# ZhenlongYuan/DVP-MVS

Hardware: AMD Instinct MI355X
Metric: Mpixels/sec/PatchMatch-iteration (higher is better)
Workload: dtype f32

## Files before the change

__graft_entry__.py:

```python
import importlib
import os
import subprocess
import sys

ROOT = os.path.dirname(os.path.abspath(__file__))
if ROOT not in sys.path:
    sys.path.insert(0, ROOT)


def build() -> None:
    subprocess.check_call(["make", "-s", "-C", os.path.join(ROOT, "dvp-mvs_amd", "csrc")])
    host = os.path.join(ROOT, "dvp-mvs_amd", "host")
    if os.path.exists(os.path.join(host, "Makefile")):
        subprocess.check_call(["make", "-s", "-C", host])
    subprocess.check_call(["make", "-s", "-C", os.path.join(ROOT, "oracle")])
    subprocess.check_call(["make", "-s", "-C", os.path.join(ROOT, "tests", "emul")])
    subprocess.check_call(["make", "-s", "-C", os.path.join(ROOT, "tests", "sweep_host")])
    subprocess.check_call(["make", "-s", "-C", os.path.join(ROOT, "tests", "host")])
    subprocess.check_call(["make", "-s", "-C", os.path.join(ROOT, "tests", "half16")])
    subprocess.check_call(["make", "-s", "-C", os.path.join(ROOT, "tests", "jpeg_host")])
    subprocess.check_call(["make", "-s", "-C", os.path.join(ROOT, "tests", "edges_host")])
    subprocess.check_call(["make", "-s", "-C", os.path.join(ROOT, "tests", "viewclean_host")])
    subprocess.check_call(["make", "-s", "-C", os.path.join(ROOT, "tests", "labels_host")])
    subprocess.check_call(["make", "-s", "-C", os.path.join(ROOT, "tests", "pyramid_host")])
    subprocess.check_call(["make", "-s", "-C", os.path.join(ROOT, "tests", "prior_host")])
    subprocess.check_call(["make", "-s", "-C", os.path.join(ROOT, "tests", "reuse_host")])
    subprocess.check_call(["make", "-s", "-C", os.path.join(ROOT, "tests", "devmem_host")])
    subprocess.check_call(["make", "-s", "-C", os.path.join(ROOT, "tests", "jpeg_dec_host")])
    subprocess.check_call(["make", "-s", "-C", os.path.join(ROOT, "tests", "convert_host")])
    subprocess.check_call(["make", "-s", "-C", os.path.join(ROOT, "tests", "undistort_host")])
    subprocess.check_call(["make", "-s", "-C", os.path.join(ROOT, "tests", "cloudeval_host")])
    pkg = importlib.import_module("dvp-mvs_amd")
    lib = pkg.get_capi().lib()
    missing = [s for s in pkg.get_capi().EXPORTS + pkg.get_capi().EXPORTS_WITH_DIGITS if not hasattr(lib, s)]
    if missing:
        raise RuntimeError("libdvp_mvs_hip.so lacks symbols: %s" % missing)


def smoke() -> None:
    import numpy as np
    pkg = importlib.import_module("dvp-mvs_amd")
    synth, capi = pkg.synth, pkg.get_capi()
    from oracle import oracle as O
    W, H, S = 96, 64, 3
    sc = synth.make_scene(W, H, S)
    p = synth.default_params(S + 1, max_iterations=1, state=synth.FIRST_INIT, use_APD=0)
    p["depth_min"] = np.float32(2.5) * np.float32(0.6)
    p["depth_max"] = np.float32(6.5) * np.float32(1.2)
    state = dict(planes=np.zeros((H * W, 4), np.float32), edge=sc["edge"], label=sc["label"],
                 radius=np.full(H * W, 5, np.int32))
# ... 21 lines not shown
```

dvp-mvs_amd/csrc/dvp_ctx.hpp:

```cpp
#ifndef DVP_CTX_HPP_
#define DVP_CTX_HPP_

#include "dvp_jpeg_enc.h"
#include "dvp_edges_run.h"
#include "dvp_viewclean_run.h"
#include "dvp_prior_run.h"
#include <cstdlib>
#include <string>
#include <vector>
#include <cstdio>
#include <mutex>
#include <condition_variable>
#include <initializer_list>

struct EventPair { int stage; hipEvent_t a, b; };
enum { EV_TOTAL = -1, EV_ITER_LOOP = -2 };

struct dvp_ctx {
	int device = 0;
	FormSwitches sw;
	int W = 0, H = 0, NI = 0, pitch = 0;
	size_t L = 0;
	hipStream_t stream = nullptr;
	bool cand_mask_fits = true;
	uint8_t* cand_mask = nullptr;
	unsigned *cand_list = nullptr, *cand_n = nullptr;
	uint32_t* sel_snap = nullptr;
	hipStream_t side = nullptr;
	hipEvent_t side_fork = nullptr, side_join = nullptr;
	Dev d{};
	std::vector<void*> allocs;
	float* images = nullptr;
	uint8_t* images8 = nullptr;
	int* images8_flag = nullptr;
	bool images8_ok = false;
	uint32_t* images16 = nullptr;
	bool images16_ok = false;
	float* image_stage = nullptr;
	float* depths = nullptr;
	uint32_t* edge_bits = nullptr;
	uint32_t* strong_bits = nullptr;
	uint32_t* strong_bits_t = nullptr;
	int* edge_sat = nullptr;
	DvpCamera* cameras = nullptr; ViewConst* views = nullptr; int* sector_taps = nullptr; int* sector_start = nullptr;
	f4* planes = nullptr; f4* planes_snap = nullptr; f4* fit_planes = nullptr;
	int* search_pos = nullptr;
	float* slot_costs = nullptr;
	float* strong_rec = nullptr;
	float* reuse_costs = nullptr; PlaneKey* reuse_keys = nullptr; ReuseHdr* reuse_hdr = nullptr;
	bool reuse_fits = true;
	uint32_t reuse_epoch = 0;
	bool split_fits = true;
	f4* sweep_rec = nullptr; float* sweep_cost = nullptr; float* sweep_pc = nullptr;
	bool sweep_fits = true;
	int sweep_band_rows = 0;
	float* costs = nullptr; float* costs_snap = nullptr; float* complex_ = nullptr;
	uint32_t* selected_views = nullptr;
	uint8_t* view_weight = nullptr; uint8_t* weak_info = nullptr; uint8_t* weak_reliable = nullptr; uint8_t* edge = nullptr;
	s2* label_stop = nullptr; s2* weak_nearest_strong = nullptr; s2* neighbours = nullptr; s2* gn_points = nullptr; int* gn_count = nullptr; s2* candidate = nullptr; s2* edge_neigh = nullptr; s2* label_boundary = nullptr;
	int* neighbours_map = nullptr; int* label = nullptr; int* radius = nullptr;
	unsigned long long* eval_counter = nullptr;
	float* scratch_out = nullptr;
	size_t weak_alloc = 0;
	AnchorRec* anchor_tab = nullptr;
	size_t anchor_tab_alloc = 0;
	bool anchor_tab_valid = false;
	bool anchor_tab_fits = true;
	WeakRec* weak_rec = nullptr; f2* weak_ctab = nullptr; float* weak_ev = nullptr;
	size_t weak_phase_alloc = 0;
	bool weak_phase_fits = true;
	int* weak_list = nullptr;
	size_t weak_list_alloc = 0;
	int* weak_counts = nullptr;
	int* weak_totals_host = nullptr;
	uint8_t* coarse = nullptr;
	uint8_t* maps_out = nullptr;
	hipStream_t copy = nullptr;
	uint8_t* maps_host = nullptr;
	std::mutex dl_m;
	std::condition_variable dl_cv;
	bool dl_busy = false;
	bool dl_fetching = false;
	size_t coarse_alloc = 0;
	uint8_t* pv_bgr[3] = { nullptr, nullptr, nullptr };
	dvpjpeg::Encoder pv_enc[3];
	unsigned long long* pv_total = nullptr;
	hipEvent_t pv_done = nullptr;
	hipStream_t pv_copy = nullptr;
// ... 52 lines not shown
		if (c->allocs[i] == (void*)*p) { c->allocs[i] = c->allocs.back(); c->allocs.pop_back(); break; }
	(void)hipFree((void*)*p);
	*p = nullptr;
}

struct AllocReq { void** p; size_t bytes; bool zero; };
template <class T>
static AllocReq areq(T** p, size_t bytes, bool zero = false) { return { reinterpret_cast<void**>(p), bytes, zero }; }

static void bump_reuse_epoch(dvp_ctx* c) {
	if (++c->reuse_epoch == 0) {
		if (c->reuse_hdr) (void)hipMemsetAsync(c->reuse_hdr, 0, c->L * sizeof(ReuseHdr), c->stream);
		c->reuse_epoch = 1;
	}
	c->d.reuse_epoch = c->reuse_epoch;
}

static size_t img16_plane_bytes(int W, int H) { return (size_t)img16_tiles_x(W) * img16_tiles_y(H) * 128; }

static bool anchor_table_off(const dvp_ctx* c) { return c->sw.anchor_tab_off || !c->anchor_tab_fits; }

static void sync_dev_struct(dvp_ctx* c) {
	Dev& d = c->d;
	d.width = c->W; d.height = c->H; d.num_images = c->NI; d.pitch = c->pitch;
	d.org = kImgPad * c->pitch + kImgPad;
	d.plane_stride = (size_t)c->pitch * (c->H + 2 * kImgPad);
	d.images = c->images; d.images8 = c->images8_ok ? c->images8 : nullptr; d.img8_tiles_x = img8_tiles_x(c->W); d.img8_plane_bytes = (size_t)img8_tiles_x(c->W) * img8_tiles_y(c->H) * 128;
	d.images16 = c->images16_ok ? c->images16 : nullptr; d.img16_tiles_x = img16_tiles_x(c->W); d.img16_plane_bytes = img16_plane_bytes(c->W, c->H);
	d.depths = c->depths; d.cameras = c->cameras; d.views = c->views; d.sector_taps = c->sector_taps; d.sector_start = c->sector_start;
	d.search_pos = c->search_pos;
	d.sweep_px0 = 0; d.sweep_row0 = 0; d.sweep_row1 = 0;
	d.sweep_all_slots = c->sw.sweep_all_slots ? 1 : 0;
	d.sweep_rec = c->sweep_rec; d.sweep_cost = c->sweep_cost; d.sweep_pc = c->sweep_pc; d.slot_costs = c->slot_costs; d.strong_rec = c->strong_rec; d.half_w = (c->W + 1) / 2;
	d.reuse_costs = c->reuse_costs; d.reuse_keys = c->reuse_keys; d.reuse_hdr = c->reuse_hdr; d.reuse_epoch = c->reuse_epoch;
	d.planes = c->planes; d.planes_snap = c->planes_snap; d.costs = c->costs; d.costs_snap = c->costs_snap;
	d.selected_views = c->selected_views; d.view_weight = c->view_weight; d.weak_info = c->weak_info;
	d.weak_reliable = c->weak_reliable; d.weak_nearest_strong = c->weak_nearest_strong;
	d.anchor_tab = (anchor_table_off(c) || !c->anchor_tab_valid) ? nullptr : c->anchor_tab; d.neighbours_map = c->neighbours_map; d.neighbours = c->neighbours; d.gn_points = c->gn_points; d.gn_count = c->gn_count; d.fit_planes = c->fit_planes;
	d.candidate = c->candidate; d.edge = c->edge; d.edge_bits = c->edge_bits; d.strong_bits = c->strong_bits; d.strong_bits_t = c->strong_bits_t; d.edge_sat = c->edge_sat; d.sat_cells_x = sat_cells(c->W); d.sat_cells_y = sat_cells(c->H); d.edge_tiles_x = edge_tiles_x(c->W); d.edge_neigh = c->edge_neigh; d.label = c->label;
	d.label_boundary = c->label_boundary; d.label_stop = c->label_stop; d.complex_ = c->complex_; d.radius = c->radius;
	d.weak_list = c->weak_list;
	d.weak_rec = c->weak_rec; d.weak_ctab = c->weak_ctab; d.weak_ev = c->weak_ev;
	d.eval_counter = c->profiling ? c->eval_counter : nullptr;
}

static int ensure_images16(dvp_ctx* c) {
	if (c->images16) return 0;
	return dalloc(c, &c->images16, img16_plane_bytes(c->W, c->H) / 4 * c->NI, false);
}

static int set_device(dvp_ctx* c) {
	HIP_TRY(c, hipSetDevice(c->device));
	return 0;
}

static size_t alloc_group_or_fall_back(dvp_ctx* c, std::initializer_list<AllocReq> reqs, const char* hook, bool* fits, const char* msg, double gb, size_t retry_bytes = 0) {
	void* got[4] = { nullptr, nullptr, nullptr, nullptr };
	const AllocReq* r = reqs.begin();
	const size_t n = reqs.size();
	size_t first = r[0].bytes;
	bool ok = n <= 4 && !(hook && getenv(hook));
	for (size_t i = 0; i < n && ok; ++i) {
		if (!r[i].p) continue;
		ok = hipMalloc(&got[i], r[i].bytes) == hipSuccess;
		if (!ok && i == 0 && retry_bytes) { (void)hipGetLastError(); first = retry_bytes; ok = hipMalloc(&got[0], first) == hipSuccess; }
		if (!ok) got[i] = nullptr;
// ... 22 lines not shown
```

dvp-mvs_amd/csrc/dvp_dev.hpp:

```cpp
#ifndef DVP_DEV_HPP_
#define DVP_DEV_HPP_

#include <stdint.h>
#include <math.h>
#include <float.h>
#include <string.h>
#include "../../include/dvp_mvs.h"
#include "dvp_forms.hpp"

#if defined(__HIPCC__)
#include <hip/hip_runtime.h>
#define DVP_HD __host__ __device__ __forceinline__
#define DVP_HD_NOINLINE __host__ __device__ __noinline__
#else
#define DVP_HD inline
#define DVP_HD_NOINLINE inline
#endif
#ifndef DVP_STREAM_HINTS
#define DVP_STREAM_HINTS 3
#endif
#if defined(__HIP_DEVICE_COMPILE__)
#define DVP_NT_STORE(bit, p, v) do { if ((DVP_STREAM_HINTS) & (bit)) __builtin_nontemporal_store((v), (p)); else *(p) = (v); } while (0)
#define DVP_NT_LOAD(bit, p) (((DVP_STREAM_HINTS) & (bit)) ? __builtin_nontemporal_load(p) : *(p))
#else
// ... 60 lines not shown
	f4* planes;
	const f4* planes_snap;
	float* costs;
	const float* costs_snap;
	uint32_t* selected_views;
	uint8_t* view_weight;
	uint8_t* weak_info;
	uint8_t* weak_reliable;
	s2* weak_nearest_strong;
	const int* neighbours_map;
	s2* neighbours;
	s2* gn_points;
	int* gn_count;
	f4* fit_planes;
	s2* candidate;
	AnchorRec* anchor_tab;
	WeakRec* weak_rec;
	f2* weak_ctab;
	float* weak_ev;
	const uint8_t* edge;
	int* search_pos;
	float* slot_costs;
	float* strong_rec;
	float* reuse_costs;
	PlaneKey* reuse_keys;
	ReuseHdr* reuse_hdr;
	uint32_t reuse_epoch;
	f4* sweep_rec;
	float* sweep_cost;
	float* sweep_pc;
	int sweep_px0;
	int sweep_row0, sweep_row1;
	int sweep_all_slots;
	int half_w;
	uint32_t* edge_bits;
	int edge_tiles_x;
	uint32_t* strong_bits;
	uint32_t* strong_bits_t;
	int* edge_sat;
	int sat_cells_x, sat_cells_y;
	s2* edge_neigh;
	const int* label;
	s2* label_boundary;
	s2* label_stop;
	float* complex_;
	int* radius;
	const int* weak_list;
	int weak_black, weak_red;
	unsigned long long* eval_counter;
};

#define DVP_MIN(a, b) ((a) > (b) ? (b) : (a))
#define DVP_MAX(a, b) ((a) < (b) ? (b) : (a))

DVP_HD float dvp_expf(float x) {
	if (!(x > -103.0f)) return (x != x) ? x : 0.0f;
	if (x > 88.72f) return INFINITY;
	const float n = rintf(x * 1.44269504088896341f);
	float r = fmaf(n, -0.693359375f, x);
	r = fmaf(n, 2.12194440e-4f, r);
	float p = 1.9875691500e-4f;
	p = fmaf(p, r, 1.3981999507e-3f);
	p = fmaf(p, r, 8.3334519073e-3f);
	p = fmaf(p, r, 4.1665795894e-2f);
	p = fmaf(p, r, 1.6666665459e-1f);
	p = fmaf(p, r, 5.0000001201e-1f);
// ... 543 lines not shown
```

dvp-mvs_amd/csrc/dvp_engine.hip:

```cpp
#include "dvp_kernels.hpp"
#include "dvp_ctx.hpp"
#ifdef DVP_PROBE
#include "dvp_probe.inc"
#endif
#include "dvp_pyramid_run.h"
#include <cstring>
#include <thread>
#include <chrono>
#include <algorithm>
#include <cmath>

extern "C" {

int dvp_ctx_create(int device, int width, int height, int num_images, dvp_ctx** out) {
	if (!out) return 1;
	*out = nullptr;
	if (width <= 0 || height <= 0 || num_images < 2 || num_images > DVP_MAX_IMAGES || width > 32767 || height > 32767) {
		g_create_error = "dvp_ctx_create: bad dimensions (2 <= num_images <= 32, sizes <= 32767: short2 pixel coordinates)";
		return 1;
	}
	{
		const unsigned long long pitch = ((unsigned long long)width + 2 * kImgPad + 63) / 64 * 64;
		if (pitch * ((unsigned long long)height + 2 * kImgPad) * 8ull >= (1ull << 32)) {
			g_create_error = "dvp_ctx_create: image too large (a padded row-pair plane must stay below 4 GiB)";
// ... 499 lines not shown
	if (alloc_group_or_fall_back(c, { areq(&c->weak_rec, cap * sizeof(WeakRec)), areq(&c->weak_ctab, cap * kTaps * kTaps * sizeof(f2)), areq(&c->weak_ev, cap * 8 * S * sizeof(float)) },
			"DVP_TEST_WEAK_PHASE_ALLOC_FAIL", &c->weak_phase_fits, "dvp: no room for the phased weak update's hand-over buffers (%.2f GB); using the one-wave kernel\n", (double)cap * (sizeof(WeakRec) + 288 + 32 * S) / 1e9))
		c->weak_phase_alloc = cap;
	return 0;
}

static void ensure_strong_reuse_buffers(dvp_ctx* c) {
	if (c->reuse_costs || !c->sw.strong_reuse || !c->reuse_fits || strong_form(c->sw, c->NI - 1, c->split_fits, false, 0).kernel != STRONG_SPLIT) return;
	const size_t L = c->L, vec = (size_t)kSlotCount * (c->NI - 1) * L * sizeof(float) + 64 ;
	const size_t Lh = (size_t)((c->W + 1) / 2) * c->H;
	alloc_group_or_fall_back(c, { areq(&c->reuse_costs, vec), areq(&c->reuse_keys, L * kSlotCount * sizeof(PlaneKey)), areq(&c->reuse_hdr, L * sizeof(ReuseHdr), true),
			c->strong_rec ? AllocReq{} : areq(&c->strong_rec, (size_t)SR_FIELDS * Lh * sizeof(*c->strong_rec)) },
		"DVP_TEST_REUSE_ALLOC_FAIL", &c->reuse_fits, "dvp: no room for the strong update's plane cache (%.1f GB); every visit evaluates all its planes\n", (double)(vec + L * (kSlotCount * sizeof(PlaneKey) + sizeof(ReuseHdr))) / 1e9);
}
static void ensure_strong_split_buffers(dvp_ctx* c) {
	if (c->slot_costs || strong_form(c->sw, c->NI - 1, c->split_fits, false, 0).kernel != STRONG_SPLIT) return;
	if (!getenv("DVP_TEST_SPLIT_ALLOC_FAIL")) {
		ensure_strong_reuse_buffers(c);
		if (c->reuse_costs) return;
	}
	const size_t Lh = (size_t)((c->W + 1) / 2) * c->H;
	alloc_group_or_fall_back(c, { areq(&c->slot_costs, (size_t)kSlotCount * (c->NI - 1) * Lh * sizeof(*c->slot_costs) + 64 ),
			areq(&c->strong_rec, (size_t)SR_FIELDS * Lh * sizeof(*c->strong_rec)) },
		"DVP_TEST_SPLIT_ALLOC_FAIL", &c->split_fits, "dvp: no room for the split strong update's cost buffer (%.1f GB); using the monolithic kernel\n", (double)kSlotCount * (c->NI - 1) * Lh * 4 / 1e9);
}
static void ensure_sweep_buffers(dvp_ctx* c) {
	if (c->sweep_cost || !c->sw.sweep_split || !c->sweep_fits) return;
	const size_t L = c->L;
	c->sweep_band_rows = sweep_band_rows(c->sw, c->W, c->H, c->NI - 1);
	const size_t band_px = c->sweep_band_rows > 0 ? (size_t)c->sweep_band_rows * c->W : L;
	alloc_group_or_fall_back(c, { areq(&c->sweep_rec, 2 * L * sizeof(f4)), areq(&c->sweep_pc, 61 * L * sizeof(float)), areq(&c->sweep_cost, sweep_cost_floats(band_px, c->NI - 1) * sizeof(float)) },
		"DVP_TEST_SWEEP_ALLOC_FAIL", &c->sweep_fits, "dvp: no room for the view-compacted DepthToWeak's cost buffer (%.1f GB); using the fused kernel\n", (double)(c->NI - 1) * kSweepFields * L * 4 / 1e9);
}


#define DVP_PICK(NAME, SUF) (c->d.sampler ? NAME##_exact##SUF : NAME##SUF)
#define DVP_PICK_FMT(NAME, TAIL) (fmt == 1 ? DVP_PICK(NAME, _u8##TAIL) : (fmt == 2 ? DVP_PICK(NAME, _f16##TAIL) : DVP_PICK(NAME, TAIL)))

static LaunchArgs make_args(const LaunchGeom& g, int colour, int iter) {
	LaunchArgs a;
	a.tiles_x = g.tiles_x; a.tiles = g.tiles; a.rows = g.rows; a.half = g.half ? 1 : 0;
	a.colour = colour; a.iter = iter;
	return a;
}

static void launch_gen_candidates(dvp_ctx* c, hipStream_t stream, const Dev& d, unsigned blocks, const LaunchArgs& a, const unsigned* list = nullptr, const unsigned* n_list = nullptr) {
	const bool all = gen_candidates_all_views(d);
	const dim3 grid(blocks, all ? (unsigned)((c->NI - 1 + kCandGroup - 1) / kCandGroup) : (unsigned)(c->NI - 1)), block(256);
	if (list) hipLaunchKernelGGL(all ? dvp_gen_candidates_views_list : dvp_gen_candidates_list, grid, block, 0, stream, d, list, n_list);
	else hipLaunchKernelGGL(all ? dvp_gen_candidates_views : dvp_gen_candidates, grid, block, 0, stream, d, a);
}

static int launch_strong_prep(dvp_ctx* c, const LaunchGeom& g, const LaunchArgs& a) {
	EventPair prep;
	prep.stage = DVP_ST_STRONG_PREP;
	HIP_TRY(c, hipEventCreate(&prep.a));
	HIP_TRY(c, hipEventCreate(&prep.b));
	HIP_TRY(c, hipEventRecord(prep.a, c->stream));
	HIP_TRY(c, hipMemcpyAsync(c->planes_snap, c->planes, c->L * 16, hipMemcpyDeviceToDevice, c->stream));
	HIP_TRY(c, hipMemcpyAsync(c->costs_snap, c->costs, c->L * 4, hipMemcpyDeviceToDevice, c->stream));
	ensure_strong_split_buffers(c);
	hipLaunchKernelGGL(dvp_strong_search, dim3(g.grid()), dim3(256), 0, c->stream, c->d, a);
	if (strong_form(c->sw, c->NI - 1, c->split_fits, c->d.reuse_hdr != nullptr, 0).plan) hipLaunchKernelGGL(dvp_strong_plan, dim3(g.grid()), dim3(256), 0, c->stream, c->d, a);
	HIP_TRY(c, hipGetLastError());
	HIP_TRY(c, hipEventRecord(prep.b, c->stream));
	c->events.push_back(prep);
// ... 72 lines not shown
	if (stage == DVP_ST_FIND_NEAREST_STRONG) HIP_TRY(c, hipMemsetAsync(c->weak_nearest_strong, 0xFF, c->L * sizeof(s2), c->stream));
	if (stage == DVP_ST_RANSAC_FIT) HIP_TRY(c, hipMemcpyAsync(c->fit_planes, c->planes, c->L * 16, hipMemcpyDeviceToDevice, c->stream));
	ListArgs la;
	la.iter = iter;
	la.covered_rows = 2 * make_geom(c->W, c->H, true).rows;
	la.base = (stage == DVP_ST_WEAK_UPDATE && colour == 1) ? c->d.weak_black : 0;
	la.count = (stage == DVP_ST_WEAK_UPDATE) ? (colour == 0 ? c->d.weak_black : (colour == 1 ? c->d.weak_red : c->d.weak_black + c->d.weak_red)) : c->d.weak_black + c->d.weak_red;
	if (la.count <= 0) return 0;
	const dim3 lg((la.count + 255) / 256);
	switch (stage) {
	case DVP_ST_FIND_NEAREST_STRONG: hipLaunchKernelGGL(DVP_PICK(dvp_find_nearest_strong_list, ), lg, block, 0, c->stream, c->d, la); break;
	case DVP_ST_GEN_NEIGHBOURS:
		if (c->sw.gn_wave) hipLaunchKernelGGL(dvp_gen_neighbours_search, dim3((la.count + 3) / 4), block, 0, c->stream, c->d, la);
		else hipLaunchKernelGGL(dvp_gen_neighbours_list, lg, block, 0, c->stream, c->d, la);
		hipLaunchKernelGGL(dvp_gen_neighbours_fit, dim3(la.count), dim3(64), 0, c->stream, c->d, la);
		break;
	case DVP_ST_NEIGHBOUR_UPDATE: hipLaunchKernelGGL(DVP_PICK(dvp_neighbour_update_list, ), lg, block, 0, c->stream, c->d, la); break;
	case DVP_ST_RANSAC_FIT:
		if (c->sw.ransac_wave) hipLaunchKernelGGL(dvp_ransac_fit_plane_wave, dim3(la.count), dim3(64), 0, c->stream, c->d, la);
		else hipLaunchKernelGGL(DVP_PICK(dvp_ransac_fit_plane_list, ), lg, block, 0, c->stream, c->d, la);
		break;
	case DVP_ST_WEAK_UPDATE:
		if (launch_weak_update(c, la)) return 1;
		break;
	}
	HIP_TRY(c, hipGetLastError());
	return 0;
}

static int launch_sweeps(dvp_ctx* c, const LaunchGeom& g, const LaunchArgs& a, bool fused) {
	const dim3 grid(g.grid()), block(256);
	if (sweep_form(c->sw, fused, c->d.params, c->sweep_fits, c->W, c->H).kernel == SWEEP_PASSES) ensure_sweep_buffers(c);
	const SweepForm f = sweep_form(c->sw, fused, c->d.params, c->sweep_fits, c->W, c->H);
	if (f.kernel == SWEEP_PASSES) {
		LaunchArgs s0 = a, s1 = a, sb = a;
		s0.iter = 0; s1.iter = 1; sb.iter = kSweepBorderOnly;
		const int etx = (c->W + 63) / 64, ety = (c->H + kSweepRows - 1) / kSweepRows;
		s0.tiles_x = s1.tiles_x = etx; s0.tiles = s1.tiles = etx * ety;
		const dim3 egrid((unsigned)(etx * ety), (unsigned)(c->NI - 1));
		hipLaunchKernelGGL(dvp_sweep_prepare, grid, block, 0, c->stream, c->d, a);
		const int band_rows = c->sweep_band_rows > 0 ? c->sweep_band_rows : c->H;
		for (int row0 = 0; row0 < c->H; row0 += band_rows) {
			Dev db = c->d;
			LaunchArgs b0 = s0, b1 = s1;
			dim3 bgrid = egrid;
			b0.rows = b1.rows = 0;
			if (c->sweep_band_rows > 0) {
				const int row1 = std::min(c->H, row0 + band_rows);
				db.sweep_px0 = row0 * c->W; db.sweep_row0 = row0; db.sweep_row1 = row1;
				const int bty = (row1 - row0 + kSweepRows - 1) / kSweepRows;
				b0.rows = b1.rows = row0 / kSweepRows;
				b0.tiles = b1.tiles = etx * bty;
				bgrid = dim3((unsigned)(etx * bty), (unsigned)(c->NI - 1));
			}
			const auto eval = c->sw.sweep_all_slots ? DVP_PICK(dvp_sweep_eval, _all) : DVP_PICK(dvp_sweep_eval, );
			hipLaunchKernelGGL(eval, bgrid, dim3(64), 0, c->stream, db, b0);
			hipLaunchKernelGGL(dvp_sweep_decide1, grid, block, 0, c->stream, db, a);
			if (f.second_eval) hipLaunchKernelGGL(eval, bgrid, dim3(64), 0, c->stream, db, b1);
			hipLaunchKernelGGL(dvp_sweep_decide2, grid, block, 0, c->stream, db, a);
		}
		if (f.border_kernel) {
			const long long frame = 12ll * c->W + 12ll * (c->H - 12);
			hipLaunchKernelGGL(DVP_PICK(dvp_sweep_border, ), dim3((unsigned)((frame + 63) / 64)), dim3(64), 0, c->stream, c->d, sb);
		}
		else hipLaunchKernelGGL(DVP_PICK(dvp_depth_to_weak_refine, ), grid, block, 0, c->stream, c->d, sb);
	}
	else if (f.kernel == SWEEP_FUSED) hipLaunchKernelGGL(DVP_PICK(dvp_depth_to_weak_refine, ), grid, block, 0, c->stream, c->d, a);
	else hipLaunchKernelGGL(DVP_PICK(dvp_depth_to_weak, ), grid, block, 0, c->stream, c->d, a);
	HIP_TRY(c, hipGetLastError());
	return 0;
}

static int launch_pixel_site(dvp_ctx* c, int stage, const LaunchGeom& g, const LaunchArgs& a, bool fused) {
	const dim3 grid(g.grid()), block(256);
	if (stage == DVP_ST_GEN_EDGE_INFORM && c->d.params.use_edge) {
		hipLaunchKernelGGL(dvp_edge_rays, dim3((c->W + c->H + 255) / 256, 8), dim3(256), 0, c->stream, c->d, 0);
		HIP_TRY(c, hipGetLastError());
	}
	if (stage == DVP_ST_GEN_EDGE_INFORM && c->d.params.use_label && c->d.weak_count > 0) {
		if (!c->label_stop) {
			if (dalloc(c, &c->label_stop, c->L * 8, false)) return 1;
			sync_dev_struct(c);
		}
		hipLaunchKernelGGL(dvp_edge_rays, dim3((c->W + c->H + 255) / 256, 8), dim3(256), 0, c->stream, c->d, 1);
		HIP_TRY(c, hipGetLastError());
	}
// ... 34 lines not shown
	case DVP_ST_DEPTH_TO_WEAK: r = launch_sweeps(c, g, a, fused); break;
	default: r = launch_pixel_site(c, stage, g, a, fused); break;
	}
	if (r) return 1;
	HIP_TRY(c, hipEventRecord(ep.b, c->stream));
	c->events.push_back(ep);
	if (c->profiling) {
		unsigned long long n = 0;
		HIP_TRY(c, hipMemcpyAsync(&n, c->eval_counter, 8, hipMemcpyDeviceToHost, c->stream));
		HIP_TRY(c, hipStreamSynchronize(c->stream));
		c->timings.ncc_evals[stage] += n;
	}
	return 0;
}

int dvp_run_stage(dvp_ctx* c, int stage, int iter, int colour) {
	if (set_device(c)) return 1;
	return launch_stage(c, stage, iter, colour);
}

static int ensure_edge_buffers(dvp_ctx* c, int slots) {
	if (dvpedge::scratch_reserve(c->eg, c->L)) { c->error = "dvp_edge_map: out of device memory"; return 1; }
	for (int k = 0; k < slots; ++k) {
		dvp_ctx::EdgeSlot& sl = c->eg_slot[k];
		if (sl.map.reserve(c->L)) { c->error = "dvp_edge_map: out of device memory"; return 1; }
		if (!sl.done && hipEventCreateWithFlags(&sl.done, hipEventDisableTiming) != hipSuccess) { (void)hipGetLastError(); sl.done = nullptr; c->error = "dvp_edge_map: hipEventCreate failed"; return 1; }
	}
	return 0;
}

int dvp_ctx_reserve(dvp_ctx* c, int weak_pixels, int flags) {
	if (set_device(c)) return 1;
	if (flags & 1) ensure_strong_split_buffers(c);
	if (flags & 2) ensure_sweep_buffers(c);
	if ((flags & 4) && !c->sw.no_images8 && !c->sw.no_images16 && ensure_images16(c)) return 1;
	if ((flags & 8) && ensure_edge_buffers(c, 2)) return 1;
	if ((flags & 16) && dvpvc::scratch_reserve(c->vc, c->L, c->NI - 1)) { c->error = "dvp_ctx_reserve: out of device memory (view clean-up)"; return 1; }
	if (weak_pixels > 0) {
		const size_t wc = std::min<size_t>((size_t)weak_pixels, c->L);
		if (grow_anchor_table(c, wc)) return 1;
		if (c->anchor_tab && grow_weak_phase_buffers(c, wc)) return 1;
		c->anchor_tab_valid = false;
	}
	return 0;
}

int dvp_synchronize(dvp_ctx* c) {
	if (set_device(c)) return 1;
	HIP_TRY(c, hipStreamSynchronize(c->stream));
	return 0;
}

int dvp_run_patchmatch(dvp_ctx* c) {
	c->anchor_tab_valid = false;
	bump_reuse_epoch(c);
	if (set_device(c)) return 1;
	EventPair tot, itl;
	tot.stage = EV_TOTAL; itl.stage = EV_ITER_LOOP;
	HIP_TRY(c, hipEventCreate(&tot.a)); HIP_TRY(c, hipEventCreate(&tot.b));
	HIP_TRY(c, hipEventCreate(&itl.a)); HIP_TRY(c, hipEventCreate(&itl.b));
	HIP_TRY(c, hipEventRecord(tot.a, c->stream));
	const bool side_work = c->d.weak_count > 0;
	if (candidates_masked(c->sw, c->d.weak_count, c->L, c->cand_mask_fits) && !c->cand_mask)
		alloc_group_or_fall_back(c, { areq(&c->cand_mask, c->L), areq(&c->cand_list, c->L * 4), areq(&c->cand_n, 4), areq(&c->sel_snap, (c->L + c->W) * 4) },
			nullptr, &c->cand_mask_fits, nullptr, 0.0);
	const bool masked = candidates_masked(c->sw, c->d.weak_count, c->L, c->cand_mask_fits);
	if (side_work && !masked) {
// ... 416 lines not shown
```

dvp-mvs_amd/csrc/dvp_forms.hpp:

```cpp
#ifndef DVP_FORMS_HPP_
#define DVP_FORMS_HPP_

#include "../../include/dvp_mvs.h"
#include <cmath>
#include <cstddef>
#include <cstdio>
#include <cstdlib>

namespace dvp {

constexpr int kNarrowViews = 8;
constexpr int kGrp = 4, kGrpWide = 2;
#ifndef DVP_SWEEP_ROWS
#define DVP_SWEEP_ROWS 14
#endif
constexpr int kSweepRows = DVP_SWEEP_ROWS;
constexpr int kSweepFields = 73;
constexpr int sweep_window(const DvpParams& P) { int cw = P.weak_peak_radius + 1; if (cw < 5) cw = 5; if (cw > 30) cw = 30; return cw; }
constexpr size_t sweep_cost_floats(size_t L, int S) { return ((L + 63) / 64) * 64 * (size_t)S * kSweepFields; }
constexpr bool sweep_slot_read(int cw, int pd, bool all_slots) { return all_slots || cw == 30 || (pd > -30 && pd < 30); }

inline bool env_flag(const char* name, bool unset) { const char* e = getenv(name); return e ? atoi(e) != 0 : unset; }

struct FormSwitches {
	bool no_images8 = false, no_images16 = false;
	bool strong_split = true, strong_reuse = true;
	bool refine_lanes = true, eval_items = true;
	int strong_wide = 0;
	bool sweep_split = true, sweep_force = false;
	bool sweep_all_slots = false;
	double sweep_band_gb = 0.0;
	bool anchor_tab_off = false;
	bool gn_wave = false, ransac_wave = false;
	int cand_mask_mode = -1;
	bool weak_phased = true, weak_split_colours = false;
	int weak_phased_min = 8192;
	int weak_run[4] = { 64, 256, 1024, 1024 }, weak_group[4] = { 1, 4, 4, 2 };
};
inline FormSwitches read_form_switches() {
	FormSwitches s;
	s.no_images8 = getenv("DVP_NO_IMAGES8") != nullptr;
	s.no_images16 = getenv("DVP_NO_IMAGES16") != nullptr;
	s.strong_split = env_flag("DVP_STRONG_SPLIT", true);
	s.strong_reuse = env_flag("DVP_STRONG_REUSE", true);
	s.refine_lanes = env_flag("DVP_REFINE_LANES", true);
	s.eval_items = env_flag("DVP_EVAL_ITEMS", true);
	if (const char* e = getenv("DVP_STRONG_WIDE")) { const int v = atoi(e); s.strong_wide = v == 0 ? 0 : (v == 2 ? 2 : 1); }
	if (const char* e = getenv("DVP_SWEEP_SPLIT")) { s.sweep_split = atoi(e) != 0; s.sweep_force = atoi(e) == 2; }
	s.sweep_all_slots = env_flag("DVP_SWEEP_ALL_SLOTS", false);
	if (const char* e = getenv("DVP_SWEEP_BAND_GB")) s.sweep_band_gb = atof(e);
	s.anchor_tab_off = !env_flag("DVP_WEAK_ANCHOR_TAB", true);
	s.gn_wave = env_flag("DVP_GN_WAVE", false);
	s.ransac_wave = env_flag("DVP_RANSAC_WAVE", false);
	if (const char* e = getenv("DVP_CAND_MASK")) s.cand_mask_mode = atoi(e) != 0 ? 1 : 0;
	s.weak_phased = env_flag("DVP_WEAK_PHASED", true);
	if (const char* e = getenv("DVP_WEAK_PHASED_MIN")) s.weak_phased_min = atoi(e);
	int g[4];
	if (const char* e = getenv("DVP_WEAK_RUNS"))
		if (sscanf(e, "%d,%d,%d,%d", &g[0], &g[1], &g[2], &g[3]) == 4)
			for (int i = 0; i < 4; ++i) s.weak_run[i] = g[i] < 1 ? 1 : g[i];
	if (const char* e = getenv("DVP_WEAK_GROUPS"))
		if (sscanf(e, "%d,%d,%d,%d", &g[0], &g[1], &g[2], &g[3]) == 4)
			for (int i = 0; i < 4; ++i) s.weak_group[i] = g[i] < 1 ? 1 : (g[i] > kGrp ? kGrp : g[i]);
	s.weak_split_colours = getenv("DVP_WEAK_SPLIT_COLOURS") != nullptr;
	return s;
}

inline int image_format(const FormSwitches& s, unsigned inexact) {
	return (inexact == 0 && !s.no_images8) ? 1 : ((inexact == 1 && !s.no_images8 && !s.no_images16) ? 2 : 0);
}

enum StrongKernel { STRONG_SPLIT, STRONG_MONO_V8, STRONG_MONO_V16, STRONG_MONO };
struct StrongForm {
	StrongKernel kernel;
	bool eval_items;
	int decide;
	bool refine_lanes;
	bool plan;
};
inline StrongForm strong_form(const FormSwitches& s, int S, bool split_fits, bool have_reuse_hdr, unsigned long long image_set_bytes) {
	const bool wide = s.strong_wide != 0 && S > 16 && S <= 31;
	if (!(s.strong_split && split_fits && (S <= 16 || wide))) return { S <= kNarrowViews ? STRONG_MONO_V8 : (S <= 16 ? STRONG_MONO_V16 : STRONG_MONO), false, 0, false, false };
	const int bracket = (wide || s.strong_wide == 2) ? 32 : (S <= 4 ? 4 : S <= 6 ? 6 : S <= 8 ? 8 : S <= 10 ? 10 : S <= 12 ? 12 : 16);
	return { STRONG_SPLIT, s.eval_items, bracket, s.refine_lanes && image_set_bytes < (1ull << 32), have_reuse_hdr };
}

enum WeakKernel { WEAK_PHASED, WEAK_WAVE, WEAK_WAVE_NOTAB };
struct WeakForm {
	WeakKernel kernel;
	int group[4], run[4];
};
inline WeakForm weak_form(const FormSwitches& s, bool table_present, bool phase_fits, int count) {
	WeakForm f{};
	const bool phased = s.weak_phased && phase_fits && (count >= s.weak_phased_min || s.weak_phased_min <= 0);
	f.kernel = !table_present ? WEAK_WAVE_NOTAB : (phased ? WEAK_PHASED : WEAK_WAVE);
	for (int i = 0; i < 4; ++i) {
		const int cap = i == 0 ? kGrpWide : kGrp;
		f.group[i] = s.weak_group[i] < cap ? s.weak_group[i] : cap;
		f.run[i] = s.weak_run[i];
	}
	return f;
}
inline bool weak_joins_colours(const FormSwitches& s, bool table_fits, bool phase_fits) {
	return s.weak_phased && phase_fits && !s.anchor_tab_off && table_fits && !s.weak_split_colours;
}

enum SweepKernel { SWEEP_PASSES, SWEEP_FUSED, SWEEP_SEPARATE };
struct SweepForm {
	SweepKernel kernel;
	bool second_eval;
	bool border_kernel;
};
inline SweepForm sweep_form(const FormSwitches& s, bool fused, const DvpParams& P, bool sweep_fits, int W, int H) {
	if (fused && s.sweep_split && sweep_fits && (P.geom_consistency || s.sweep_force)) return { SWEEP_PASSES, sweep_window(P) < 30, W >= 12 && H >= 12 };
	return { fused ? SWEEP_FUSED : SWEEP_SEPARATE, false, false };
}
inline int sweep_band_rows(const FormSwitches& s, int W, int H, int S) {
	if (!(s.sweep_band_gb > 0.0)) return 0;
	const int bands = (int)std::ceil((double)sweep_cost_floats((size_t)W * H, S) * sizeof(float) / (s.sweep_band_gb * 1e9));
	if (bands <= 1) return 0;
	const int rows = ((H + bands - 1) / bands + kSweepRows - 1) / kSweepRows * kSweepRows;
	return rows < H ? rows : 0;
}

inline bool candidates_masked(const FormSwitches& s, int weak_count, size_t L, bool mask_fits) {
	return weak_count > 0 && mask_fits && (s.cand_mask_mode == 1 || (s.cand_mask_mode < 0 && (size_t)weak_count * 25 < L));
}

}
#endif
```

dvp-mvs_amd/csrc/dvp_kernels.hpp:

```cpp
#ifndef DVP_KERNELS_HPP_
#define DVP_KERNELS_HPP_

#include "dvp_stages.hpp"
#include <hip/hip_runtime.h>

using namespace dvp;

struct LaunchArgs {
	int tiles_x, tiles, rows, half, colour, iter;
};

template <int STAGE, int SMP, int MV = 32>
__device__ __forceinline__ void stage_body(const Dev& d, const LaunchArgs& a) {
	const int lane = threadIdx.x & 63;
	const int wave = threadIdx.x >> 6;
	int px, py;
	unsigned long long n = 0;
	__shared__ f2 lds_tab[stage_uses_tab(STAGE) ? kTaps * kTaps * 256 : 1];
	const PatchTab tab{&lds_tab[stage_uses_tab(STAGE) ? threadIdx.x : 0], 256};
	if (block_to_pixel(blockIdx.x, lane, wave, a.tiles_x, a.tiles, a.rows, a.half, a.colour, d.width, d.height, &px, &py))
		run_pixel<STAGE, SMP, MV>(d, px, py, a.iter, d.eval_counter ? &n : nullptr, tab);
	if (d.eval_counter && n) atomicAdd(d.eval_counter, n);
}

// ... 236 lines not shown
		}
	}
	if (d.eval_counter && cnt) atomicAdd(d.eval_counter, cnt);
}
template <int SMP>
__device__ __forceinline__ void sweep_border_body(const Dev& d, const LaunchArgs& a) {
	__shared__ f2 lds_tab[kTaps * kTaps * 64];
	const PatchTab tab{&lds_tab[threadIdx.x], 64};
	const int W = d.width, H = d.height;
	const long long t = (long long)blockIdx.x * 64 + threadIdx.x;
	int px, py;
	if (t < 12ll * W) {
		const int r = (int)(t / W);
		px = (int)(t - (long long)r * W);
		py = r < 6 ? r : H - 12 + r;
	} else {
		const long long u = t - 12ll * W;
		const int r = (int)(u / 12), cidx = (int)(u - 12ll * r);
		if (r >= H - 12) return;
		py = 6 + r;
		px = cidx < 6 ? cidx : W - 12 + cidx;
	}
	unsigned long long n = 0;
	run_pixel<kStageSweeps, SMP>(d, px, py, kSweepBorderOnly, d.eval_counter ? &n : nullptr, tab);
	if (d.eval_counter && n) atomicAdd(d.eval_counter, n);
}
extern "C" __global__ void __launch_bounds__(64, DVP_LB_HEAVY) dvp_sweep_border(const Dev d, const LaunchArgs a) { sweep_border_body<0>(d, a); }
extern "C" __global__ void __launch_bounds__(64, DVP_LB_HEAVY) dvp_sweep_border_exact(const Dev d, const LaunchArgs a) { sweep_border_body<1>(d, a); }
extern "C" __global__ void __launch_bounds__(64, DVP_LB_HEAVY) dvp_sweep_eval(const Dev d, const LaunchArgs a) { sweep_eval_body<0, false>(d, a); }
extern "C" __global__ void __launch_bounds__(64, DVP_LB_HEAVY) dvp_sweep_eval_exact(const Dev d, const LaunchArgs a) { sweep_eval_body<1, false>(d, a); }
extern "C" __global__ void __launch_bounds__(64, DVP_LB_HEAVY) dvp_sweep_eval_all(const Dev d, const LaunchArgs a) { sweep_eval_body<0, true>(d, a); }
extern "C" __global__ void __launch_bounds__(64, DVP_LB_HEAVY) dvp_sweep_eval_exact_all(const Dev d, const LaunchArgs a) { sweep_eval_body<1, true>(d, a); }

DVP_KERNEL_LIST(dvp_find_nearest_strong_list, DVP_ST_FIND_NEAREST_STRONG, 1)
extern "C" __global__ void __launch_bounds__(256) dvp_gen_neighbours_list(const Dev d, const ListArgs a) {
	__shared__ s2 pts[kGnDirSlots * 256];
	const int t = list_block(blockIdx.x, gridDim.x, kListRun) * 256 + threadIdx.x;
	if (t >= a.count) return;
	const int center = d.weak_list[a.base + t];
	const int py = center / d.width, px = center - py * d.width;
	gen_neighbours_px(d, px, py, pts + threadIdx.x, 256);
}
DVP_KERNEL_LIST(dvp_neighbour_update_list, DVP_ST_NEIGHBOUR_UPDATE, 1)
DVP_KERNEL_LIST(dvp_ransac_fit_plane_list, DVP_ST_RANSAC_FIT, 1)
extern "C" __global__ void __launch_bounds__(64) dvp_ransac_fit_plane_wave(const Dev d, const ListArgs a) {
	__shared__ RansacShared sh[1];
	const int t = list_block(blockIdx.x, gridDim.x, kWaveRun * 4);
	if (t >= a.count) return;
	const int center = d.weak_list[a.base + t];
	const int py = center / d.width, px = center - py * d.width;
	ransac_fit_plane_wave(d, px, py, a.iter, sh[0]);
}

template <int SMP, int FMT, int TAB>
__device__ __forceinline__ void weak_wave_body(const Dev& d, const ListArgs& a) {
	__shared__ WeakSharedT<TAB> sh[1];
	const int wave = 0;
	const int t = list_block(blockIdx.x, gridDim.x, kWaveRun * 4);
	if (t >= a.count) return;
	const int center = d.weak_list[a.base + t];
	const int py = center / d.width, px = center - py * d.width;
	if (py >= a.covered_rows) return;
	if (d.weak_info[center] != DVP_WEAK) return;
	unsigned long long n = 0;
	weak_update_wave<SMP, FMT, TAB>(d, px, py, a.iter, d.eval_counter ? &n : nullptr, sh[wave]);
	if (d.eval_counter && n) atomicAdd(d.eval_counter, n);
// ... 459 lines not shown
```

dvp-mvs_amd/csrc/dvp_stages.hpp:

```cpp
#ifndef DVP_STAGES_HPP_
#define DVP_STAGES_HPP_

#include "dvp_edge_inform.hpp"
#include "dvp_ransac.hpp"
#include "dvp_weak_wave.hpp"
#include "dvp_weak_phased.hpp"
#include "dvp_sweep.hpp"
#include <vector>
#include <cmath>

namespace dvp {

struct LaunchGeom {
	int tiles_x, tiles_y, tiles;
	int rows;
	bool half;
	int grid() const { return tiles; }
};
inline LaunchGeom make_geom(int W, int H, bool half) {
	LaunchGeom g;
	g.half = half;
	g.rows = half ? ((H / 2) + 15) / 16 * 16 : H;
	g.tiles_x = (W + 63) / 64;
	g.tiles_y = (g.rows + 3) / 4;
	g.tiles = g.tiles_x * g.tiles_y;
	return g;
}

DVP_HD bool block_to_pixel(int block, int lane, int wave, int tiles_x, int tiles, int rows, int half, int colour,
	int W, int H, int* px, int* py) {
	if (block >= tiles) return false;
	const int tiles_y = tiles / tiles_x;
	const int per_strip = 8 * tiles_y;
	const int st = block / per_strip;
	const int rem = block - st * per_strip;
	const int w_last = tiles_x - st * 8;
	int ty, tx;
	if (w_last >= 8) {
		ty = rem >> 3;
		tx = st * 8 + (rem & 7);
// ... 123 lines not shown
```

Baseline: 61.73.

## Compact sweep evaluation into per-view (pixel) lists before launching eval

```diff
diff --git a/__graft_entry__.py b/__graft_entry__.py
--- a/__graft_entry__.py
+++ b/__graft_entry__.py
@@ -16,6 +16,7 @@
     subprocess.check_call(["make", "-s", "-C", os.path.join(ROOT, "oracle")])
     subprocess.check_call(["make", "-s", "-C", os.path.join(ROOT, "tests", "emul")])
     subprocess.check_call(["make", "-s", "-C", os.path.join(ROOT, "tests", "sweep_host")])
+    subprocess.check_call(["make", "-s", "-C", os.path.join(ROOT, "tests", "sweep_list_host")])
     subprocess.check_call(["make", "-s", "-C", os.path.join(ROOT, "tests", "host")])
     subprocess.check_call(["make", "-s", "-C", os.path.join(ROOT, "tests", "half16")])
     subprocess.check_call(["make", "-s", "-C", os.path.join(ROOT, "tests", "jpeg_host")])
diff --git a/dvp-mvs_amd/csrc/dvp_ctx.hpp b/dvp-mvs_amd/csrc/dvp_ctx.hpp
--- a/dvp-mvs_amd/csrc/dvp_ctx.hpp
+++ b/dvp-mvs_amd/csrc/dvp_ctx.hpp
@@ -54,6 +54,9 @@
 	f4* sweep_rec = nullptr; float* sweep_cost = nullptr; float* sweep_pc = nullptr;
 	bool sweep_fits = true;
 	int sweep_band_rows = 0;
+	uint32_t* sweep_list = nullptr; int* sweep_list_counts = nullptr;
+	int sweep_list_cap = 0, sweep_list_tiles = 0;
+	bool sweep_list_fits = true;
 	float* costs = nullptr; float* costs_snap = nullptr; float* complex_ = nullptr;
 	uint32_t* selected_views = nullptr;
 	uint8_t* view_weight = nullptr; uint8_t* weak_info = nullptr; uint8_t* weak_reliable = nullptr; uint8_t* edge = nullptr;
@@ -172,6 +175,8 @@
 	d.sweep_px0 = 0; d.sweep_row0 = 0; d.sweep_row1 = 0;
 	d.sweep_all_slots = c->sw.sweep_all_slots ? 1 : 0;
 	d.sweep_rec = c->sweep_rec; d.sweep_cost = c->sweep_cost; d.sweep_pc = c->sweep_pc; d.slot_costs = c->slot_costs; d.strong_rec = c->strong_rec; d.half_w = (c->W + 1) / 2;
+	d.sweep_list = c->sweep_list; d.sweep_list_counts = c->sweep_list_counts; d.sweep_list_cap = c->sweep_list_cap;
+	d.sweep_list_n = c->sweep_list_counts ? c->sweep_list_counts + (size_t)(c->NI - 1) * c->sweep_list_tiles : nullptr;
 	d.reuse_costs = c->reuse_costs; d.reuse_keys = c->reuse_keys; d.reuse_hdr = c->reuse_hdr; d.reuse_epoch = c->reuse_epoch;
 	d.planes = c->planes; d.planes_snap = c->planes_snap; d.costs = c->costs; d.costs_snap = c->costs_snap;
 	d.selected_views = c->selected_views; d.view_weight = c->view_weight; d.weak_info = c->weak_info;
diff --git a/dvp-mvs_amd/csrc/dvp_dev.hpp b/dvp-mvs_amd/csrc/dvp_dev.hpp
--- a/dvp-mvs_amd/csrc/dvp_dev.hpp
+++ b/dvp-mvs_amd/csrc/dvp_dev.hpp
@@ -116,6 +116,10 @@
 	int sweep_px0;
 	int sweep_row0, sweep_row1;
 	int sweep_all_slots;
+	uint32_t* sweep_list;
+	int* sweep_list_n;
+	int* sweep_list_counts;
+	int sweep_list_cap;
 	int half_w;
 	uint32_t* edge_bits;
 	int edge_tiles_x;
diff --git a/dvp-mvs_amd/csrc/dvp_engine.hip b/dvp-mvs_amd/csrc/dvp_engine.hip
--- a/dvp-mvs_amd/csrc/dvp_engine.hip
+++ b/dvp-mvs_amd/csrc/dvp_engine.hip
@@ -555,6 +555,15 @@
 	alloc_group_or_fall_back(c, { areq(&c->sweep_rec, 2 * L * sizeof(f4)), areq(&c->sweep_pc, 61 * L * sizeof(float)), areq(&c->sweep_cost, sweep_cost_floats(band_px, c->NI - 1) * sizeof(float)) },
 		"DVP_TEST_SWEEP_ALLOC_FAIL", &c->sweep_fits, "dvp: no room for the view-compacted DepthToWeak's cost buffer (%.1f GB); using the fused kernel\n", (double)(c->NI - 1) * kSweepFields * L * 4 / 1e9);
 }
+static void ensure_sweep_list_buffers(dvp_ctx* c) {
+	if (c->sweep_list || !c->sweep_cost || !c->sw.sweep_list || !c->sweep_list_fits) return;
+	const size_t S = (size_t)c->NI - 1;
+	const int band_rows = c->sweep_band_rows > 0 ? c->sweep_band_rows : c->H;
+	c->sweep_list_cap = band_rows * c->W;
+	c->sweep_list_tiles = ((c->W + 63) / 64) * ((band_rows + kSweepRows - 1) / kSweepRows);
+	alloc_group_or_fall_back(c, { areq(&c->sweep_list, S * (size_t)c->sweep_list_cap * sizeof(uint32_t)), areq(&c->sweep_list_counts, (S * c->sweep_list_tiles + (S + 2) / 3 * 3) * sizeof(int)) },
+		"DVP_TEST_SWEEP_LIST_ALLOC_FAIL", &c->sweep_list_fits, "dvp: no room for the sweep passes' (pixel, view) lists (%.2f GB); evaluating tile by tile\n", (double)S * c->sweep_list_cap * 4 / 1e9);
+}
 
 
 #define DVP_PICK(NAME, SUF) (c->d.sampler ? NAME##_exact##SUF : NAME##SUF)
@@ -693,7 +702,10 @@
 	const dim3 grid(g.grid()), block(256);
 	if (sweep_form(c->sw, fused, c->d.params, c->sweep_fits, c->W, c->H).kernel == SWEEP_PASSES) ensure_sweep_buffers(c);
 	const SweepForm f = sweep_form(c->sw, fused, c->d.params, c->sweep_fits, c->W, c->H);
+	if (sweep_eval_form(c->sw, f, c->sweep_list_fits) == SWEEP_EVAL_LISTS) ensure_sweep_list_buffers(c);
 	if (f.kernel == SWEEP_PASSES) {
+		const bool lists = sweep_eval_form(c->sw, f, c->sweep_list_fits) == SWEEP_EVAL_LISTS;
+		const auto list_eval = c->sw.sweep_all_slots ? DVP_PICK(dvp_sweep_eval_list, _all) : DVP_PICK(dvp_sweep_eval_list, );
 		LaunchArgs s0 = a, s1 = a, sb = a;
 		s0.iter = 0; s1.iter = 1; sb.iter = kSweepBorderOnly;
 		const int etx = (c->W + 63) / 64, ety = (c->H + kSweepRows - 1) / kSweepRows;
@@ -713,6 +725,21 @@
 				b0.rows = b1.rows = row0 / kSweepRows;
 				b0.tiles = b1.tiles = etx * bty;
 				bgrid = dim3((unsigned)(etx * bty), (unsigned)(c->NI - 1));
+			}
+			if (lists) {
+				const int S = c->NI - 1, T = b0.tiles;
+				const dim3 tgrid((unsigned)((T + 3) / 4)), lgrid((unsigned)sweep_list_grid(c->sweep_list_cap, kSweepListRounds), (unsigned)S);
+				for (int stage = 0; stage < (f.second_eval ? 2 : 1); ++stage) {
+					const LaunchArgs& bs = stage ? b1 : b0;
+					hipLaunchKernelGGL(dvp_sweep_list_counts, tgrid, block, 0, c->stream, db, bs);
+					for (int v0 = 0; v0 < S; v0 += 3)
+						hipLaunchKernelGGL(dvp_scan3, dim3(3), dim3(1024), 0, c->stream, db.sweep_list_counts, v0 * T, std::min(v0 + 1, S) * T, std::min(v0 + 2, S) * T, std::min(v0 + 3, S) * T, db.sweep_list_n + v0);
+					hipLaunchKernelGGL(dvp_sweep_list_fill, tgrid, block, 0, c->stream, db, bs);
+					hipLaunchKernelGGL(list_eval, lgrid, dim3(64), 0, c->stream, db, bs);
+					if (stage == 0) hipLaunchKernelGGL(dvp_sweep_decide1, grid, block, 0, c->stream, db, a);
+				}
+				hipLaunchKernelGGL(dvp_sweep_decide2, grid, block, 0, c->stream, db, a);
+				continue;
 			}
 			const auto eval = c->sw.sweep_all_slots ? DVP_PICK(dvp_sweep_eval, _all) : DVP_PICK(dvp_sweep_eval, );
 			hipLaunchKernelGGL(eval, bgrid, dim3(64), 0, c->stream, db, b0);
@@ -813,7 +840,7 @@
 int dvp_ctx_reserve(dvp_ctx* c, int weak_pixels, int flags) {
 	if (set_device(c)) return 1;
 	if (flags & 1) ensure_strong_split_buffers(c);
-	if (flags & 2) ensure_sweep_buffers(c);
+	if (flags & 2) { ensure_sweep_buffers(c); ensure_sweep_list_buffers(c); }
 	if ((flags & 4) && !c->sw.no_images8 && !c->sw.no_images16 && ensure_images16(c)) return 1;
 	if ((flags & 8) && ensure_edge_buffers(c, 2)) return 1;
 	if ((flags & 16) && dvpvc::scratch_reserve(c->vc, c->L, c->NI - 1)) { c->error = "dvp_ctx_reserve: out of device memory (view clean-up)"; return 1; }
diff --git a/dvp-mvs_amd/csrc/dvp_forms.hpp b/dvp-mvs_amd/csrc/dvp_forms.hpp
--- a/dvp-mvs_amd/csrc/dvp_forms.hpp
+++ b/dvp-mvs_amd/csrc/dvp_forms.hpp
@@ -30,6 +30,7 @@
 	bool sweep_split = true, sweep_force = false;
 	bool sweep_all_slots = false;
 	double sweep_band_gb = 0.0;
+	bool sweep_list = true;
 	bool anchor_tab_off = false;
 	bool gn_wave = false, ransac_wave = false;
 	int cand_mask_mode = -1;
@@ -49,6 +50,7 @@
 	if (const char* e = getenv("DVP_SWEEP_SPLIT")) { s.sweep_split = atoi(e) != 0; s.sweep_force = atoi(e) == 2; }
 	s.sweep_all_slots = env_flag("DVP_SWEEP_ALL_SLOTS", false);
 	if (const char* e = getenv("DVP_SWEEP_BAND_GB")) s.sweep_band_gb = atof(e);
+	s.sweep_list = env_flag("DVP_SWEEP_LIST", true);
 	s.anchor_tab_off = !env_flag("DVP_WEAK_ANCHOR_TAB", true);
 	s.gn_wave = env_flag("DVP_GN_WAVE", false);
 	s.ransac_wave = env_flag("DVP_RANSAC_WAVE", false);
@@ -115,6 +117,10 @@
 	if (fused && s.sweep_split && sweep_fits && (P.geom_consistency || s.sweep_force)) return { SWEEP_PASSES, sweep_window(P) < 30, W >= 12 && H >= 12 };
 	return { fused ? SWEEP_FUSED : SWEEP_SEPARATE, false, false };
 }
+enum SweepEval { SWEEP_EVAL_TILES, SWEEP_EVAL_LISTS };
+inline SweepEval sweep_eval_form(const FormSwitches& s, const SweepForm& f, bool list_fits) {
+	return (f.kernel == SWEEP_PASSES && s.sweep_list && list_fits) ? SWEEP_EVAL_LISTS : SWEEP_EVAL_TILES;
+}
 inline int sweep_band_rows(const FormSwitches& s, int W, int H, int S) {
 	if (!(s.sweep_band_gb > 0.0)) return 0;
 	const int bands = (int)std::ceil((double)sweep_cost_floats((size_t)W * H, S) * sizeof(float) / (s.sweep_band_gb * 1e9));
diff --git a/dvp-mvs_amd/csrc/dvp_kernels.hpp b/dvp-mvs_amd/csrc/dvp_kernels.hpp
--- a/dvp-mvs_amd/csrc/dvp_kernels.hpp
+++ b/dvp-mvs_amd/csrc/dvp_kernels.hpp
@@ -292,6 +292,80 @@
 extern "C" __global__ void __launch_bounds__(64, DVP_LB_HEAVY) dvp_sweep_eval_all(const Dev d, const LaunchArgs a) { sweep_eval_body<0, true>(d, a); }
 extern "C" __global__ void __launch_bounds__(64, DVP_LB_HEAVY) dvp_sweep_eval_exact_all(const Dev d, const LaunchArgs a) { sweep_eval_body<1, true>(d, a); }
 
+extern "C" __global__ void __launch_bounds__(256) dvp_sweep_list_counts(const Dev d, const LaunchArgs a) {
+	const int lane = threadIdx.x & 63;
+	const int t = blockIdx.x * 4 + (threadIdx.x >> 6);
+	if (t >= a.tiles) return;
+	const int S = d.params.num_images - 1;
+	int tx, ty;
+	sweep_list_tile(t, a.tiles_x, a.tiles / a.tiles_x, &tx, &ty);
+	ty += a.rows;
+	const int x = tx * 64 + lane;
+	int cnt = 0;
+	for (int r = 0; r < kSweepRows; ++r) {
+		const int y = ty * kSweepRows + r;
+		const uint32_t m = (x < d.width && y < d.height) ? sweep_go_mask(d, x + y * d.width, a.iter) : 0u;
+		if (__ballot(m != 0) == 0) continue;
+		for (int v = 0; v < S; ++v) {
+			const int k = __popcll(__ballot((m >> v) & 1u));
+			if (lane == v) cnt += k;
+		}
+	}
+	if (lane < S) d.sweep_list_counts[(size_t)lane * a.tiles + t] = cnt;
+}
+extern "C" __global__ void __launch_bounds__(256) dvp_sweep_list_fill(const Dev d, const LaunchArgs a) {
+	const int lane = threadIdx.x & 63;
+	const int t = blockIdx.x * 4 + (threadIdx.x >> 6);
+	if (t >= a.tiles) return;
+	const int S = d.params.num_images - 1;
+	int tx, ty;
+	sweep_list_tile(t, a.tiles_x, a.tiles / a.tiles_x, &tx, &ty);
+	ty += a.rows;
+	const int x = tx * 64 + lane;
+	int off = lane < S ? d.sweep_list_counts[(size_t)lane * a.tiles + t] : 0;
+	for (int r = 0; r < kSweepRows; ++r) {
+		const int y = ty * kSweepRows + r;
+		const uint32_t m = (x < d.width && y < d.height) ? sweep_go_mask(d, x + y * d.width, a.iter) : 0u;
+		if (__ballot(m != 0) == 0) continue;
+		for (int v = 0; v < S; ++v) {
+			const unsigned long long b = __ballot((m >> v) & 1u);
+			sweep_list_put(d.sweep_list + (size_t)v * d.sweep_list_cap, __shfl(off, v, 64), b, lane, x, y);
+			if (lane == v) off += __popcll(b);
+		}
+	}
+}
+template <int SMP, bool ALL, int R>
+__device__ __forceinline__ void sweep_eval_list_body(const Dev& d, const LaunchArgs& a) {
+	const int lane = threadIdx.x;
+	const int v = blockIdx.y;
+	__shared__ f2 lds_tab[kTaps * kTaps * 64];
+	__shared__ DvpCamera cams[2];
+	const int n = d.sweep_list_n[v];
+	const int chunk = sweep_list_chunk((int)blockIdx.x, n, R);
+	if (chunk < 0) return;
+	const PatchTab tab{&lds_tab[lane], 64};
+	static_assert(sizeof(DvpCamera) == 112, "28 dwords");
+	if (lane < 56) {
+		const int which = lane >= 28 ? 1 : 0;
+		reinterpret_cast<uint32_t*>(&cams[which])[lane - 28 * which] = reinterpret_cast<const uint32_t*>(d.cameras + (which ? v + 1 : 0))[lane - 28 * which];
+	}
+	__syncthreads();
+	const uint32_t* list = d.sweep_list + (size_t)v * d.sweep_list_cap;
+	const int first = chunk * (64 * R), end = DVP_MIN(n, first + 64 * R);
+	unsigned long long cnt = 0;
+	for (int i0 = first; i0 < end; i0 += 64) {
+		if (i0 + lane < end) {
+			const uint32_t e = list[i0 + lane];
+			sweep_eval_px<SMP, ALL>(d, sweep_list_x(e), sweep_list_y(e), v, a.iter, tab, d.eval_counter ? &cnt : nullptr, cams);
+		}
+	}
+	if (d.eval_counter && cnt) atomicAdd(d.eval_counter, cnt);
+}
+extern "C" __global__ void __launch_bounds__(64, DVP_LB_HEAVY) dvp_sweep_eval_list(const Dev d, const LaunchArgs a) { sweep_eval_list_body<0, false, kSweepListRounds>(d, a); }
+extern "C" __global__ void __launch_bounds__(64, DVP_LB_HEAVY) dvp_sweep_eval_list_exact(const Dev d, const LaunchArgs a) { sweep_eval_list_body<1, false, kSweepListRounds>(d, a); }
+extern "C" __global__ void __launch_bounds__(64, DVP_LB_HEAVY) dvp_sweep_eval_list_all(const Dev d, const LaunchArgs a) { sweep_eval_list_body<0, true, kSweepListRounds>(d, a); }
+extern "C" __global__ void __launch_bounds__(64, DVP_LB_HEAVY) dvp_sweep_eval_list_exact_all(const Dev d, const LaunchArgs a) { sweep_eval_list_body<1, true, kSweepListRounds>(d, a); }
+
 DVP_KERNEL_LIST(dvp_find_nearest_strong_list, DVP_ST_FIND_NEAREST_STRONG, 1)
 extern "C" __global__ void __launch_bounds__(256) dvp_gen_neighbours_list(const Dev d, const ListArgs a) {
 	__shared__ s2 pts[kGnDirSlots * 256];
diff --git a/dvp-mvs_amd/csrc/dvp_stages.hpp b/dvp-mvs_amd/csrc/dvp_stages.hpp
--- a/dvp-mvs_amd/csrc/dvp_stages.hpp
+++ b/dvp-mvs_amd/csrc/dvp_stages.hpp
@@ -6,6 +6,7 @@
 #include "dvp_weak_wave.hpp"
 #include "dvp_weak_phased.hpp"
 #include "dvp_sweep.hpp"
+#include "dvp_sweep_list.hpp"
 #include <vector>
 #include <cmath>
 
diff --git a/dvp-mvs_amd/csrc/dvp_sweep_list.hpp b/dvp-mvs_amd/csrc/dvp_sweep_list.hpp
--- /dev/null
+++ b/dvp-mvs_amd/csrc/dvp_sweep_list.hpp
@@ -0,0 +1,102 @@
+#ifndef DVP_SWEEP_LIST_HPP_
+#define DVP_SWEEP_LIST_HPP_
+
+#include "dvp_sweep.hpp"
+#include <cstring>
+
+namespace dvp {
+
+#ifndef DVP_SWEEP_LIST_R
+#define DVP_SWEEP_LIST_R 2
+#endif
+constexpr int kSweepListRounds = DVP_SWEEP_LIST_R;
+
+DVP_HD uint32_t sweep_go_mask(const Dev& d, int center, int stage) {
+	const size_t L = (size_t)d.width * (size_t)d.height;
+	const int flags = (int)d.sweep_rec[L + center].w;
+	if (!(flags & (stage == 0 ? SWF_VALID : SWF_PEAK))) return 0;
+	const int S = d.params.num_images - 1;
+	uint32_t sel = d.selected_views[center];
+	if (S < 32) sel &= (1u << S) - 1u;
+	const uint8_t* vw = static_cast<const uint8_t*>(__builtin_assume_aligned(d.view_weight + (size_t)center * 32, 4));
+	uint32_t m = 0;
+	for (int q = 0; q * 4 < S; ++q) {
+		uint32_t w;
+		memcpy(&w, vw + 4 * q, 4);
+		uint32_t nz = 0;
+		for (int b = 0; b < 4; ++b) nz |= ((w >> (8 * b)) & 255u) ? 1u << b : 0u;
+		m |= nz << (4 * q);
+	}
+	return sel & m;
+}
+
+DVP_HD void sweep_list_tile(int t, int tiles_x, int tiles_y, int* tx, int* ty) {
+	const int per_strip = 8 * tiles_y;
+	const int st = t / per_strip, rem = t - st * per_strip;
+	const int w_last = tiles_x - st * 8;
+	if (w_last >= 8) { *ty = rem >> 3; *tx = st * 8 + (rem & 7); }
+	else { *ty = rem / w_last; *tx = st * 8 + (rem - *ty * w_last); }
+}
+DVP_HD uint32_t sweep_list_pack(int x, int y) { return ((uint32_t)y << 16) | (uint32_t)x; }
+DVP_HD int sweep_list_x(uint32_t e) { return (int)(e & 0xFFFFu); }
+DVP_HD int sweep_list_y(uint32_t e) { return (int)(e >> 16); }
+DVP_HD void sweep_list_put(uint32_t* list, int at, unsigned long long m, int lane, int x, int y) {
+	if ((m >> lane) & 1ull) list[at + __builtin_popcountll(m & ((1ull << lane) - 1ull))] = sweep_list_pack(x, y);
+}
+
+DVP_HD int sweep_list_grid(int cap, int rounds) { return (cap + 64 * rounds - 1) / (64 * rounds); }
+DVP_HD int sweep_list_chunk(int b, int n, int rounds) {
+	const int chunks = (n + 64 * rounds - 1) / (64 * rounds);
+	return b < chunks ? b : -1;
+}
+
+#if !defined(__HIP_DEVICE_COMPILE__)
+inline void sweep_list_counts_host(const Dev& d, int tiles_x, int tiles, int rows, int stage, int* counts) {
+	const int S = d.params.num_images - 1;
+	for (int t = 0; t < tiles; ++t) {
+		int tx, ty;
+		sweep_list_tile(t, tiles_x, tiles / tiles_x, &tx, &ty);
+		ty += rows;
+		for (int v = 0; v < S; ++v) counts[(size_t)v * tiles + t] = 0;
+		for (int r = 0; r < kSweepRows; ++r)
+			for (int lane = 0; lane < 64; ++lane) {
+				const int x = tx * 64 + lane, y = ty * kSweepRows + r;
+				const uint32_t m = (x < d.width && y < d.height) ? sweep_go_mask(d, x + y * d.width, stage) : 0u;
+				for (int v = 0; v < S; ++v) counts[(size_t)v * tiles + t] += (int)((m >> v) & 1u);
+			}
+	}
+}
+inline void sweep_list_scan_host(int S, int tiles, int* counts, int* n) {
+	for (int v = 0; v < S; ++v) {
+		int run = 0;
+		for (int t = 0; t < tiles; ++t) { const int k = counts[(size_t)v * tiles + t]; counts[(size_t)v * tiles + t] = run; run += k; }
+		n[v] = run;
+	}
+}
+inline void sweep_list_fill_host(const Dev& d, int tiles_x, int tiles, int rows, int stage, const int* offs, uint32_t* list, int cap) {
+	const int S = d.params.num_images - 1;
+	for (int t = 0; t < tiles; ++t) {
+		int tx, ty, o[32];
+		sweep_list_tile(t, tiles_x, tiles / tiles_x, &tx, &ty);
+		ty += rows;
+		for (int v = 0; v < S; ++v) o[v] = offs[(size_t)v * tiles + t];
+		for (int r = 0; r < kSweepRows; ++r) {
+			const int y = ty * kSweepRows + r;
+			uint32_t mk[64];
+			for (int lane = 0; lane < 64; ++lane) {
+				const int x = tx * 64 + lane;
+				mk[lane] = (x < d.width && y < d.height) ? sweep_go_mask(d, x + y * d.width, stage) : 0u;
+			}
+			for (int v = 0; v < S; ++v) {
+				unsigned long long m = 0;
+				for (int lane = 0; lane < 64; ++lane) m |= (unsigned long long)((mk[lane] >> v) & 1u) << lane;
+				for (int lane = 0; lane < 64; ++lane) sweep_list_put(list + (size_t)v * cap, o[v], m, lane, tx * 64 + lane, y);
+				o[v] += __builtin_popcountll(m);
+			}
+		}
+	}
+}
+#endif
+
+}
+#endif
```

Result: faster. 62.77, median of 6 (+1.7%).
